# datastax/jvector

Hardware: AMD Instinct MI355X
Metric: QPS@recall10>=0.95 (10Mx768); distances/sec as % HBM roofline (higher is better)
Workload: dtype f32

## Files before the change

jvector_amd/csrc/gs_body.h:

```cpp
#pragma once

#include <cstdint>

#include "gs_params.h"

#ifndef GS_UBR_VAR_LPS
#define GS_UBR_VAR_LPS 1
#endif

namespace jv {

struct alignas(16) gs_f4 { float x, y, z, w; };
struct alignas(16) gs_u4 { uint32_t x, y, z, w; };

GS_FN int32_t gs_float_bits(float f)
{
    int32_t b;
    __builtin_memcpy(&b, &f, 4);
    return b;
}
GS_FN float gs_bits_float(int32_t b)
{
    float f;
    __builtin_memcpy(&f, &b, 4);
// ... 60 lines not shown
    *idx_out = (int)gs_shfl((long long)bi, gs_first(who));
    return m;
}

GS_FN long long gs_scan_top2(const long long *a, int n, int *idx_out, long long *second_out)
{
    const int lane = gs_lane();
    long long best = GS_KEY_MIN, second = GS_KEY_MIN;
    int bi = -1;
    for (int i = lane; i < n; i += 256) {
        long long k[4];
#pragma unroll
        for (int u = 0; u < 4; ++u) k[u] = (i + 64 * u < n) ? a[i + 64 * u] : GS_KEY_MIN;
#pragma unroll
        for (int u = 0; u < 4; ++u) {
            if (k[u] > best) {
                second = best;
                best = k[u];
                bi = i + 64 * u;
            } else if (k[u] > second) {
                second = k[u];
            }
        }
    }
    const long long m = gs_wave_max(best);
    const int w = gs_first(gs_ballot(bi >= 0 && best == m));
    *idx_out = (int)gs_shfl((long long)bi, w);
    *second_out = gs_wave_max(lane == w ? second : best);
    return m;
}

template <int CH16>
GS_FN void gs_load_row(const uint8_t *rp, gs_u4 (&w)[CH16])
{
    const gs_u4 *r4 = reinterpret_cast<const gs_u4 *>(rp);
#pragma unroll
    for (int c = 0; c < CH16; ++c) w[c] = r4[c];
}

template <int VSF, int CH16>
GS_FN float gs_row_sum(const float *codebooks, const float *qs, const gs_u4 (&w)[CH16])
{
    float sum = 0.0f;
#pragma unroll
    for (int c = 0; c < CH16; ++c) {
        const uint32_t d[4] = {w[c].x, w[c].y, w[c].z, w[c].w};
#pragma unroll
        for (int e = 0; e < 4; ++e) {
#pragma unroll
            for (int b = 0; b < 4; ++b) {
                const int m = c * 16 + e * 4 + b;
                const uint32_t code = (d[e] >> (8 * b)) & 0xFFu;
                const gs_f4 *cp = reinterpret_cast<const gs_f4 *>(codebooks + ((int64_t)(m * 256) + code) * 8);
                const gs_f4 c0 = cp[0], c1 = cp[1];
                const float *q = qs + m * 8;
                float ent = 0.0f;
                if (VSF == 0 ) {
                    float t;
                    t = c0.x - q[0]; ent += t * t;
                    t = c0.y - q[1]; ent += t * t;
                    t = c0.z - q[2]; ent += t * t;
                    t = c0.w - q[3]; ent += t * t;
                    t = c1.x - q[4]; ent += t * t;
                    t = c1.y - q[5]; ent += t * t;
                    t = c1.z - q[6]; ent += t * t;
                    t = c1.w - q[7]; ent += t * t;
                } else {
                    ent += c0.x * q[0];
                    ent += c0.y * q[1];
                    ent += c0.z * q[2];
                    ent += c0.w * q[3];
                    ent += c1.x * q[4];
                    ent += c1.y * q[5];
                    ent += c1.z * q[6];
                    ent += c1.w * q[7];
                }
                sum += ent;
            }
        }
    }
    return sum;
}

template <int VSF>
GS_FN float gs_row_sum_any(const GsParams &p, const float *qs, const uint8_t *rp)
{
    float sum = 0.0f;
    const int M = p.M;
    if (p.sub_uniform4 > 0) {
        const int S = p.sub_uniform4;
#pragma unroll 4
        for (int m = 0; m < M; ++m) {
            const gs_f4 *cp = reinterpret_cast<const gs_f4 *>(p.codebooks + ((int64_t)m * 256 + rp[m]) * S);
            const float *q = qs + m * S;
            float ent = 0.0f;
            for (int j = 0; j < S; j += 4) {
                const gs_f4 c = cp[j >> 2];
                if (VSF == 0 ) {
                    float t;
                    t = c.x - q[j]; ent += t * t;
                    t = c.y - q[j + 1]; ent += t * t;
                    t = c.z - q[j + 2]; ent += t * t;
                    t = c.w - q[j + 3]; ent += t * t;
                } else {
                    ent += c.x * q[j];
                    ent += c.y * q[j + 1];
                    ent += c.z * q[j + 2];
                    ent += c.w * q[j + 3];
                }
            }
            sum += ent;
        }
        return sum;
    }
#pragma unroll 2
    for (int m = 0; m < M; ++m) {
        const int S = p.sub_sizes[m];
        const float *cb = p.codebooks + p.cb_offsets[m] + (int64_t)rp[m] * S;
        const float *q = qs + p.sub_offsets[m];
        float ent = 0.0f;
        for (int j = 0; j < S; ++j) {
            if (VSF == 0 ) {
                const float t = cb[j] - q[j];
                ent += t * t;
            } else {
                ent += cb[j] * q[j];
            }
        }
        sum += ent;
    }
    return sum;
}

template <int VSF>
GS_FN float gs_lut_entry_from(const gs_f4 c0, const gs_f4 c1, const float *q);
template <int VSF>
GS_FN float gs_lut_entry(const float *codebooks, const float *qs, int m, int code)
{
    const gs_f4 *cp = reinterpret_cast<const gs_f4 *>(codebooks + ((int64_t)(m * 256) + code) * 8);
    return gs_lut_entry_from<VSF>(cp[0], cp[1], qs + m * 8);
}
template <int VSF>
GS_FN float gs_lut_entry_from(const gs_f4 c0, const gs_f4 c1, const float *q)
{
    float ent = 0.0f;
    if (VSF == 0 ) {
        float t;
        t = c0.x - q[0]; ent += t * t;
        t = c0.y - q[1]; ent += t * t;
        t = c0.z - q[2]; ent += t * t;
        t = c0.w - q[3]; ent += t * t;
        t = c1.x - q[4]; ent += t * t;
        t = c1.y - q[5]; ent += t * t;
        t = c1.z - q[6]; ent += t * t;
        t = c1.w - q[7]; ent += t * t;
    } else {
        ent += c0.x * q[0];
        ent += c0.y * q[1];
        ent += c0.z * q[2];
        ent += c0.w * q[3];
        ent += c1.x * q[4];
        ent += c1.y * q[5];
        ent += c1.z * q[6];
        ent += c1.w * q[7];
    }
    return ent;
}

template <int VSF>
GS_FN float gs_lut_entry_pk(const gs_f4 c0, const gs_f4 c1, const float *q)
{
#ifdef GS_HAVE_PK_F32
    if (VSF != 0) {
        const gs_f4 q0 = reinterpret_cast<const gs_f4 *>(q)[0], q1 = reinterpret_cast<const gs_f4 *>(q)[1];
        const gs_pk2 p01 = gs_pk2{c0.x, c0.y} * gs_pk2{q0.x, q0.y}, p23 = gs_pk2{c0.z, c0.w} * gs_pk2{q0.z, q0.w};
        const gs_pk2 p45 = gs_pk2{c1.x, c1.y} * gs_pk2{q1.x, q1.y}, p67 = gs_pk2{c1.z, c1.w} * gs_pk2{q1.z, q1.w};
        float ent = 0.0f;
        ent += p01.x;
        ent += p01.y;
        ent += p23.x;
        ent += p23.y;
        ent += p45.x;
        ent += p45.y;
        ent += p67.x;
        ent += p67.y;
        return ent;
    }
#endif
    return gs_lut_entry_from<VSF>(c0, c1, q);
}

template <int VSF>
GS_FN float gs_lut_entry_pk_q(const gs_f4 c0, const gs_f4 c1, const gs_f4 q0, const gs_f4 q1)
{
#ifdef GS_HAVE_PK_F32
    if (VSF != 0) {
        const gs_pk2 p01 = gs_pk2{c0.x, c0.y} * gs_pk2{q0.x, q0.y}, p23 = gs_pk2{c0.z, c0.w} * gs_pk2{q0.z, q0.w};
        const gs_pk2 p45 = gs_pk2{c1.x, c1.y} * gs_pk2{q1.x, q1.y}, p67 = gs_pk2{c1.z, c1.w} * gs_pk2{q1.z, q1.w};
        float ent = 0.0f;
        ent += p01.x;
        ent += p01.y;
        ent += p23.x;
        ent += p23.y;
        ent += p45.x;
        ent += p45.y;
        ent += p67.x;
        ent += p67.y;
        return ent;
    }
#endif
    const float q[8] = {q0.x, q0.y, q0.z, q0.w, q1.x, q1.y, q1.z, q1.w};
    return gs_lut_entry_from<VSF>(c0, c1, q);
}

template <int VSF, int CH16, bool FULL = false>
GS_FN float gx_row_sum(const float *lut, int lut_m, const float *codebooks, const float *qs, const gs_u4 (&w)[CH16])
{
    float sum = 0.0f;
#pragma unroll
    for (int c = 0; c < CH16; ++c) {
        const uint32_t d[4] = {w[c].x, w[c].y, w[c].z, w[c].w};
        if (FULL || c * 16 < lut_m) {
#pragma unroll
            for (int e = 0; e < 4; ++e) {
#pragma unroll
                for (int b = 0; b < 4; ++b) {
                    const int m = c * 16 + e * 4 + b;
                    const uint32_t code = (d[e] >> (8 * b)) & 0xFFu;
                    sum += lut[m * 256 + (int)code];
                }
            }
        } else {
#pragma unroll
            for (int e = 0; e < 4; ++e) {
#pragma unroll
                for (int b = 0; b < 4; ++b) {
                    const int m = c * 16 + e * 4 + b;
                    const uint32_t code = (d[e] >> (8 * b)) & 0xFFu;
                    sum += gs_lut_entry<VSF>(codebooks, qs, m, (int)code);
                }
            }
        }
    }
    return sum;
}

struct alignas(8) gs_u2 { uint32_t x, y; };

template <int HW>
GS_FN void gs_load_half(const uint8_t *rp, gs_u2 (&w)[HW])
{
    const gs_u2 *r2 = reinterpret_cast<const gs_u2 *>(rp);
#pragma unroll
    for (int c = 0; c < HW; ++c) w[c] = r2[c];
}

template <int VSF, int HW, int XS = 32>
GS_FN float gs_half_entries(const float *codebooks, const float *qs, const gs_u2 (&w)[HW], int m_base, float *xw)
{
    float sum = 0.0f;
#pragma unroll
    for (int c = 0; c < HW; ++c) {
        const uint32_t d[2] = {w[c].x, w[c].y};
#pragma unroll
        for (int e = 0; e < 2; ++e) {
#pragma unroll
            for (int b = 0; b < 4; ++b) {
                const int j = c * 8 + e * 4 + b;
                const int m = m_base + j;
                const uint32_t code = (d[e] >> (8 * b)) & 0xFFu;
                const gs_f4 *cp = reinterpret_cast<const gs_f4 *>(codebooks + ((int64_t)m * 256 + code) * 8);
                const gs_f4 c0 = cp[0], c1 = cp[1];
                const float *q = qs + m * 8;
                float v = 0.0f;
                if (VSF == 0 ) {
                    float t;
                    t = c0.x - q[0]; v += t * t;
                    t = c0.y - q[1]; v += t * t;
                    t = c0.z - q[2]; v += t * t;
                    t = c0.w - q[3]; v += t * t;
                    t = c1.x - q[4]; v += t * t;
                    t = c1.y - q[5]; v += t * t;
                    t = c1.z - q[6]; v += t * t;
                    t = c1.w - q[7]; v += t * t;
                } else {
                    v += c0.x * q[0];
                    v += c0.y * q[1];
                    v += c0.z * q[2];
                    v += c0.w * q[3];
                    v += c1.x * q[4];
                    v += c1.y * q[5];
                    v += c1.z * q[6];
                    v += c1.w * q[7];
                }
                if (xw) xw[j * XS] = v;
                else sum += v;
            }
        }
    }
    return sum;
}


template <int CH16>
GS_FN void gs_ubr_load(const uint32_t *tab_q, uint32_t (&tab)[CH16 * 16])
{
    const gs_u4 *src = reinterpret_cast<const gs_u4 *>(tab_q) + gs_lane();
#pragma unroll
    for (int k = 0; k < CH16 * 4; ++k) {
        const gs_u4 v = src[k * 64];
        tab[4 * k + 0] = v.x;
        tab[4 * k + 1] = v.y;
        tab[4 * k + 2] = v.z;
        tab[4 * k + 3] = v.w;
    }
}

template <int CH16>
GS_FN int32_t gs_ubr_half(const uint32_t (&tab)[CH16 * 16], const gs_u2 (&w)[CH16], int hi, bool lower = false)
{
    int32_t acc = lower ? 0 : CH16 * 8;
    const uint32_t selbase = 0x0c0c0c00u + 2u * (uint32_t)hi;
#pragma unroll
    for (int c = 0; c < CH16; ++c) {
        const uint32_t d[2] = {w[c].x, w[c].y};
        uint32_t lo[8], up[8], sel[8];
#pragma unroll
        for (int i = 0; i < 8; ++i) {
            const int r = c * 8 + i;
            const uint32_t code = (d[i >> 2] >> (8 * (i & 3))) & 0xFFu;
            const int src = (int)(code & 63u);
            lo[i] = (uint32_t)gs_shfl32((int32_t)tab[2 * r], src);
            up[i] = (uint32_t)gs_shfl32((int32_t)tab[2 * r + 1], src);
            const uint32_t t2 = code >> 6;
            sel[i] = selbase + t2 + (t2 & 2u);
        }
#pragma unroll
        for (int i = 0; i < 8; ++i) acc += (int32_t)gs_perm(up[i], lo[i], sel[i]);
    }
    return acc;
}

template <int VSF>
GS_FN float gs_finish(float sum, float node_mag, float query_mag)
{
    if (VSF == 0) return 1.0f / (1.0f + sum);
    if (VSF == 2) {
        const float prod = node_mag * query_mag;
        sum = (float)((double)sum / gs_sqrt((double)prod));
    }
    return (1.0f + sum) / 2.0f;
}

template <int VSF>
GS_FN bool gs_bound_below(float bound_raw, float node_mag, float query_mag, float T)
{
    if (VSF == 0) return bound_raw > 0.0f && gs_finish<VSF>(bound_raw, node_mag, query_mag) < T;
    if (VSF != 2) return gs_finish<VSF>(bound_raw, node_mag, query_mag) < T;
    const float prod = node_mag * query_mag;
    if (!(prod > 0.0f) || !(prod < 3.0e38f)) return false;
    const float x = bound_raw * gs_rsq_approx(prod);
    const float ax = x < 0.0f ? -x : x;
    return x + 1e-5f * (1.0f + ax) < 2.0f * T - 1.0f;
}

template <int VSF>
GS_FN float gs_bound_score(float bound_raw, float node_mag, float query_mag)
{
    float u;
    if (VSF == 2) {
        const float prod = node_mag * query_mag;
        if (!(prod > 0.0f) || !(prod < 3.0e38f)) return __builtin_inff();
        const float x = bound_raw * gs_rsq_approx(prod);
        const float ax = x < 0.0f ? -x : x;
        u = 0.5f * (1.0f + (x + 1e-5f * (1.0f + ax)));
    } else {
        u = gs_finish<VSF>(bound_raw, node_mag, query_mag);
    }
    const float au = u < 0.0f ? -u : u;
    return u + 1e-6f * (1.0f + au);
}

template <int VSF, int M_, int LPS>
GS_FN void gs_ubr_pass(const float *codebooks, const float *qs, float *xf, const int32_t *st_nb, const float *st_mag, const uint8_t *st_code,
                       int base, int ns, float query_mag, bool ub_active, float ub_T, bool &fresh, long long &key)
{
    static_assert(M_ % LPS == 0 && (LPS == 8 || LPS == 16 || LPS == 32), "lanes per survivor");
    constexpr int SUBS = M_ / LPS;
    constexpr int RH = SUBS % 6 == 0 ? 6 : (SUBS % 4 == 0 ? 4 : SUBS);
    constexpr int QB = RH % 3 == 0 ? 3 : (RH % 2 == 0 ? 2 : 1);
    static_assert(SUBS % RH == 0 && RH % QB == 0 && RH <= 6, "whole rounds of whole batches");
    constexpr int NB = (LPS - 1) * SUBS;
    constexpr int CS = (NB + 3) & ~3;
    const int lane = gs_lane();
    const int g = lane / LPS;
    int t = lane % LPS;
    GS_OPAQUE_I32(t);
    const int j = base + g;
    const bool work = j < ns;
    float sum = 0.0f;
    if (work) {
        const int off = t * SUBS;
        const uint32_t *cw = reinterpret_cast<const uint32_t *>(st_code + j * M_ + (off & ~3));
        uint32_t d[SUBS / 4 > 3 ? SUBS / 4 : 3];
        if (SUBS % 4 == 0) {
#pragma unroll
            for (int i = 0; i < SUBS / 4; ++i) d[i] = cw[i];
        } else {
            const unsigned long long win = (unsigned long long)cw[0] | ((unsigned long long)cw[1] << 32);
            const unsigned long long sh = win >> (8 * (off & 3));
            d[0] = (uint32_t)sh;
            d[1] = (uint32_t)(sh >> 32);
            d[2] = 0u;
        }
        float v[SUBS];
#pragma unroll
        for (int h2 = 0; h2 < SUBS / RH; ++h2) {
            gs_f4 c0[RH], c1[RH];
#pragma unroll
            for (int kk = 0; kk < RH; ++kk) {
                const int k = h2 * RH + kk;
                const uint32_t code = (d[k >> 2] >> (8 * (k & 3))) & 0xFFu;
                const gs_f4 *cp = reinterpret_cast<const gs_f4 *>(codebooks + ((int64_t)((t * SUBS + k) * 256) + code) * 8);
                c0[kk] = cp[0];
                c1[kk] = cp[1];
            }
#pragma unroll
            for (int b3 = 0; b3 < RH / QB; ++b3) {
                gs_f4 q0[QB], q1[QB];
#pragma unroll
                for (int kk = 0; kk < QB; ++kk) {
                    const gs_f4 *qp = reinterpret_cast<const gs_f4 *>(qs + (t * SUBS + h2 * RH + b3 * QB + kk) * 8);
                    q0[kk] = qp[0];
                    q1[kk] = qp[1];
                }
                GS_SCHED_FENCE();
#pragma unroll
                for (int kk = 0; kk < QB; ++kk) {
                    const int k = h2 * RH + b3 * QB + kk;
                    v[k] = gs_lut_entry_pk_q<VSF>(c0[b3 * QB + kk], c1[b3 * QB + kk], q0[kk], q1[kk]);
                }
                GS_SCHED_FENCE();
            }
        }
        if (t == 0) {
#pragma unroll
            for (int k = 0; k < SUBS; ++k) sum += v[k];
        } else {
#pragma unroll
            for (int k = 0; k < SUBS; ++k) xf[g * CS + (t - 1) * SUBS + k] = v[k];
        }
    }
    gs_barrier();
    fresh = work && t == 0;
    key = 0;
    if (fresh) {
        const gs_f4 *col = reinterpret_cast<const gs_f4 *>(xf + g * CS);
        constexpr int NW = CS / 4;
        constexpr int EB = NW % 7 == 0 ? 7 : 8;
#pragma unroll
        for (int b7 = 0; b7 < (NW + EB - 1) / EB; ++b7) {
            gs_f4 e4[EB];
#pragma unroll
            for (int i = 0; i < EB; ++i)
                if (b7 * EB + i < NW) e4[i] = col[b7 * EB + i];
            GS_SCHED_FENCE();
#pragma unroll
            for (int i = 0; i < EB; ++i) {
                const int w0 = (b7 * EB + i) * 4;
                if (w0 + 0 < NB) sum += e4[i].x;
                if (w0 + 1 < NB) sum += e4[i].y;
                if (w0 + 2 < NB) sum += e4[i].z;
                if (w0 + 3 < NB) sum += e4[i].w;
            }
            GS_SCHED_FENCE();
        }
        const float sc = gs_finish<VSF>(sum, st_mag[j], query_mag);
        key = gs_key(st_nb[j], sc);
        if (ub_active && sc < ub_T) fresh = false;
    }
}

GS_FN bool gs_visit(int32_t *tab, uint32_t mask, int shift, int32_t node)
{
    uint32_t h = ((uint32_t)node * 0x9E3779B1u) >> shift;
    for (;;) {
        const int32_t old = gs_cas(tab + h, -1, node);
        if (old == -1) return true;
        if (old == node) return false;
        h = (h + 1) & mask;
    }
}

struct GsVis1 {
    uint32_t *w;
    uint32_t bmask;
    uint32_t idmask;
    int rbits;
};

GS_FN int gs_v1_bucket(uint32_t *bw, uint32_t mine)
{
    for (;;) {
        const uint32_t w0 = bw[0], w1 = bw[1];
        const uint32_t e0 = w0 & 0xFFFFu, e1 = w0 >> 16, e2 = w1 & 0xFFFFu, e3 = w1 >> 16;
        if (e0 == mine || e1 == mine || e2 == mine || e3 == mine) return 0;
        const int slot = e0 == 0xFFFFu ? 0 : (e1 == 0xFFFFu ? 1 : (e2 == 0xFFFFu ? 2 : (e3 == 0xFFFFu ? 3 : -1)));
        if (slot < 0) return 2;
        const uint32_t w = slot < 2 ? w0 : w1;
        const int sh = (slot & 1) * 16;
        const uint32_t want = (w & ~(0xFFFFu << sh)) | (mine << sh);
        if (gs_lds_cas(bw + (slot >> 1), w, want) == w) return 1;
    }
}

GS_FN int gs_visit1(const GsVis1 &t, int32_t node)
{
    const uint32_t rmask = (1u << t.rbits) - 1u;
    const uint32_t h0 = ((uint32_t)node * 0x9E3779B1u) & t.idmask;
    const int r = gs_v1_bucket(t.w + 2u * ((h0 >> t.rbits) & t.bmask), h0 & rmask);
    if (r != 2) return r;
    const uint32_t h1 = ((uint32_t)node * 0x85EBCA6Bu) & t.idmask;
    return gs_v1_bucket(t.w + 2u * ((h1 >> t.rbits) & t.bmask), (1u << t.rbits) | (h1 & rmask));
}

GS_FN const int32_t *gs_level_row(const GsLevel &L, int32_t node)
{
    if (!L.hkeys) return (node >= 0 && node < L.count) ? L.nbrs + (int64_t)node * L.degree : nullptr;
    uint32_t h = ((uint32_t)node * 0x9E3779B1u) >> L.hshift;
    for (;;) {
        const int32_t k = L.hkeys[h];
        if (k == node) return L.nbrs + (int64_t)L.hvals[h] * L.degree;
        if (k == -1) return nullptr;
        h = (h + 1) & L.hmask;
    }
}

struct GsState {
    long long *cand, *res, *evicted, *samp;
    long long *spill;
    int cand_n, spill_n, res_n, ev_n, res_min_idx, spill_cap;
    long long spill_max, res_min;
    int32_t status;
};

GS_FN void gs_partition(GsState &s, const GsParams &p)
{
    const int lane = gs_lane();
    const uint64_t lt = (1ull << lane) - 1ull;
    const long long mine = s.cand[(int)(((long long)lane * s.cand_n) >> 6)];
    s.samp[lane] = mine;
    gs_barrier();
    int rank = 0;
    for (int j = 0; j < 64; ++j) rank += (s.samp[j] < mine) ? 1 : 0;
    const long long pivot = gs_shfl(mine, gs_first(gs_ballot(rank == 31)));
    int new_n = 0, moved = 0;
    for (int base = 0; base < s.cand_n; base += 64) {
        const int i = base + lane;
        const bool in = i < s.cand_n;
        const long long k = in ? s.cand[i] : 0;
        const bool hi = in && k > pivot;
        const bool lo = in && !hi;
        const uint64_t mh = gs_ballot(hi), ml = gs_ballot(lo);
        if (hi) s.cand[new_n + gs_popc(mh & lt)] = k;
        if (lo) {
            const int pos = s.spill_n + moved + gs_popc(ml & lt);
            if (pos < s.spill_cap) s.spill[pos] = k;
        }
        new_n += gs_popc(mh);
        moved += gs_popc(ml);
        gs_barrier();
    }
    if (s.spill_n + moved > s.spill_cap) s.status = GS_OVERFLOW;
    s.spill_n += moved;
    s.cand_n = new_n;
    s.spill_max = pivot;
}

GS_FN void gs_refill(GsState &s, const GsParams &p)
{
    const int lane = gs_lane();
    const uint64_t lt = (1ull << lane) - 1ull;
    gs_fence();
    const int n = s.spill_n;
    if (n <= p.cand_cap / 2) {
        for (int base = 0; base < n; base += 64)
            if (base + lane < n) s.cand[base + lane] = s.spill[base + lane];
        s.cand_n = n;
        s.spill_n = 0;
        s.spill_max = GS_KEY_MIN;
        gs_barrier();
        return;
    }
    const long long mine = s.spill[(int)(((long long)lane * n) >> 6)];
    s.samp[lane] = mine;
    gs_barrier();
    int rank = 0;
    for (int j = 0; j < 64; ++j) rank += (s.samp[j] < mine) ? 1 : 0;
    int r = 63 - (int)(((long long)(p.cand_cap / 4) * 64) / n);
    r = r < 1 ? 1 : (r > 62 ? 62 : r);
    long long pivot = 0;
    int above = 0;
    for (int attempt = 0; attempt < 8; ++attempt) {
        pivot = gs_shfl(mine, gs_first(gs_ballot(rank == r)));
        above = 0;
        for (int base = 0; base < n; base += 64) above += gs_popc(gs_ballot(base + lane < n && s.spill[base + lane] > pivot));
        if (above <= p.cand_cap - 64 || r >= 62) break;
        r += (64 - r) / 2;
        if (r > 62) r = 62;
    }
    gs_barrier();
    if (above == 0 || above > p.cand_cap - 64) return;
    int nc = 0, ns = 0;
    for (int base = 0; base < n; base += 64) {
        const int i = base + lane;
        const bool in = i < n;
        const long long k = in ? s.spill[i] : 0;
        const bool hi = in && k > pivot;
        const bool lo = in && !hi;
        const uint64_t mh = gs_ballot(hi), ml = gs_ballot(lo);
        if (hi) s.cand[nc + gs_popc(mh & lt)] = k;
        if (lo) s.spill[ns + gs_popc(ml & lt)] = k;
        nc += gs_popc(mh);
        ns += gs_popc(ml);
        gs_barrier();
    }
    s.cand_n = nc;
    s.spill_n = ns;
    s.spill_max = pivot;
    gs_fence();
}

GS_FN void gs_push(GsState &s, const GsParams &p, long long key, bool has)
{
    const int lane = gs_lane();
    const uint64_t lt = (1ull << lane) - 1ull;
    bool to_lds;
    uint64_t ml;
    for (;;) {
        to_lds = has && (s.spill_n == 0 || key > s.spill_max);
        ml = gs_ballot(to_lds);
// ... 1236 lines not shown
```

jvector_amd/csrc/gs_wave_hip.h:

```cpp
#pragma once

#include <hip/hip_runtime.h>

#include <cstdint>

#define GS_FN __device__ __forceinline__
#define GS_SCHED_FENCE() __builtin_amdgcn_sched_barrier(0)
#define GS_NOINLINE __device__ __attribute__((noinline))
#define GS_LDS_AS __attribute__((address_space(3)))
#define GS_GLOBAL_AS __attribute__((address_space(1)))
__device__ __forceinline__ int gs_lane() { return (int)threadIdx.x; }
#ifdef GS_WAVE_SCOPE_BARRIER
__device__ __forceinline__ void gs_barrier()
{
    __builtin_amdgcn_fence(__ATOMIC_RELEASE, "wavefront");
    __builtin_amdgcn_wave_barrier();
    __builtin_amdgcn_fence(__ATOMIC_ACQUIRE, "wavefront");
}
#else
__device__ __forceinline__ void gs_barrier() { __syncthreads(); }
#endif
__device__ __forceinline__ int gs_tid() { return (int)threadIdx.x; }
__device__ __forceinline__ void gs_block_barrier() { __syncthreads(); }
__device__ __forceinline__ int gs_block_threads() { return (int)blockDim.x; }
__device__ __forceinline__ int32_t gs_lds_load(const int32_t *p)
{
    const int32_t v = *(const volatile __attribute__((address_space(3))) int32_t *)p;
    __asm__ volatile("s_waitcnt lgkmcnt(0)" ::: "memory");
    return v;
}
__device__ __forceinline__ void gs_lds_store(int32_t *p, int32_t v)
{
    __asm__ volatile("s_waitcnt lgkmcnt(0)" ::: "memory");
    *(volatile __attribute__((address_space(3))) int32_t *)p = v;
}
__device__ __forceinline__ int32_t gs_lds_add(int32_t *p, int32_t v)
{
    return __hip_atomic_fetch_add((__attribute__((address_space(3))) int32_t *)p, v, __ATOMIC_RELAXED, __HIP_MEMORY_SCOPE_WORKGROUP);
}
__device__ __forceinline__ void gs_spin_pause() { __builtin_amdgcn_s_sleep(1); }
__device__ __forceinline__ void gs_sched_fence() { __builtin_amdgcn_sched_barrier(0); }
__device__ __forceinline__ uint64_t gs_ballot(bool p) { return (uint64_t)__ballot(p ? 1 : 0); }
#ifdef GS_UNIFORM_SHFL
__device__ __forceinline__ long long gs_shfl(long long v, int src)
{
    const int lo = __builtin_amdgcn_readlane((int)(unsigned long long)v, src), hi = __builtin_amdgcn_readlane((int)((unsigned long long)v >> 32), src);
    return (long long)(((unsigned long long)(unsigned)hi << 32) | (unsigned long long)(unsigned)lo);
}
#define GS_HAVE_WAVE_REDUCE 1
template <bool MAX>
__device__ __forceinline__ long long gs_wave_reduce64(long long v)
{
#define JV_DPP_STEP(CTRL, ROWS)                                                                                       \
    do {                                                                                                              \
        const int lo_ = __builtin_amdgcn_update_dpp((int)(unsigned long long)v, (int)(unsigned long long)v, CTRL, ROWS, 0xf, false);              \
        const int hi_ = __builtin_amdgcn_update_dpp((int)((unsigned long long)v >> 32), (int)((unsigned long long)v >> 32), CTRL, ROWS, 0xf, false); \
        const long long o_ = (long long)(((unsigned long long)(unsigned)hi_ << 32) | (unsigned long long)(unsigned)lo_);                          \
        v = MAX ? (o_ > v ? o_ : v) : (o_ < v ? o_ : v);                                                              \
    } while (0)
    JV_DPP_STEP(0x111, 0xf);
    JV_DPP_STEP(0x112, 0xf);
    JV_DPP_STEP(0x114, 0xf);
    JV_DPP_STEP(0x118, 0xf);
    JV_DPP_STEP(0x142, 0xa);
    JV_DPP_STEP(0x143, 0xc);
#undef JV_DPP_STEP
    const int lo = __builtin_amdgcn_readlane((int)(unsigned long long)v, 63), hi = __builtin_amdgcn_readlane((int)((unsigned long long)v >> 32), 63);
    return (long long)(((unsigned long long)(unsigned)hi << 32) | (unsigned long long)(unsigned)lo);
}
__device__ __forceinline__ long long gs_wave_max(long long v) { return gs_wave_reduce64<true>(v); }
__device__ __forceinline__ long long gs_wave_min(long long v) { return gs_wave_reduce64<false>(v); }
#define GS_HAVE_WAVE_REDUCE32 1
#define JV_DPP_RED32(T, NAME, EXPR)                                                                  \
    __device__ __forceinline__ T NAME(T v)                                                           \
    {                                                                                                \
        _Pragma("unroll") for (int s_ = 0; s_ < 6; ++s_)                                             \
        {                                                                                            \
            T o_;                                                                                    \
            switch (s_) {                                                                            \
            case 0: o_ = (T)__builtin_amdgcn_update_dpp((int)v, (int)v, 0x111, 0xf, 0xf, false); break; \
            case 1: o_ = (T)__builtin_amdgcn_update_dpp((int)v, (int)v, 0x112, 0xf, 0xf, false); break; \
            case 2: o_ = (T)__builtin_amdgcn_update_dpp((int)v, (int)v, 0x114, 0xf, 0xf, false); break; \
            case 3: o_ = (T)__builtin_amdgcn_update_dpp((int)v, (int)v, 0x118, 0xf, 0xf, false); break; \
            case 4: o_ = (T)__builtin_amdgcn_update_dpp((int)v, (int)v, 0x142, 0xa, 0xf, false); break; \
            default: o_ = (T)__builtin_amdgcn_update_dpp((int)v, (int)v, 0x143, 0xc, 0xf, false); break; \
            }                                                                                        \
            v = EXPR;                                                                                \
        }                                                                                            \
        return (T)__builtin_amdgcn_readlane((int)v, 63);                                             \
    }
JV_DPP_RED32(int32_t, gs_wave_max_i32, (o_ > v ? o_ : v))
JV_DPP_RED32(int32_t, gs_wave_min_i32, (o_ < v ? o_ : v))
JV_DPP_RED32(uint32_t, gs_wave_max_u32, (o_ > v ? o_ : v))
#undef JV_DPP_RED32
__device__ __forceinline__ int32_t gs_uniform(int32_t v) { return __builtin_amdgcn_readfirstlane(v); }
#else
__device__ __forceinline__ long long gs_shfl(long long v, int src) { return __shfl(v, src, 64); }
#endif
__device__ __forceinline__ uint32_t gs_bcast32(uint32_t v, int src) { return (uint32_t)__builtin_amdgcn_readlane((int)v, src); }
__device__ __forceinline__ long long gs_shfl_xor(long long v, int m) { return __shfl_xor(v, m, 64); }
#define GS_OPAQUE_I32(x) asm volatile("" : "+v"(x))
__device__ __forceinline__ int32_t gs_shfl32(int32_t v, int src) { return __builtin_amdgcn_ds_bpermute(src << 2, v); }
#define GS_HAVE_PK_F32 1
typedef float gs_pk2 __attribute__((ext_vector_type(2)));
__device__ __forceinline__ uint32_t gs_perm(uint32_t hi, uint32_t lo, uint32_t sel) { return __builtin_amdgcn_perm(hi, lo, sel); }
__device__ __forceinline__ int32_t gs_cas(int32_t *p, int32_t expect, int32_t desired) { return atomicCAS(p, expect, desired); }
__device__ __forceinline__ uint32_t gs_lds_cas(uint32_t *p, uint32_t expect, uint32_t desired)
{
    typedef __attribute__((address_space(3))) uint32_t lds_u32;
    lds_u32 *lp = (lds_u32 *)p;
    __hip_atomic_compare_exchange_strong(lp, &expect, desired, __ATOMIC_RELAXED, __ATOMIC_RELAXED, __HIP_MEMORY_SCOPE_WORKGROUP);
    return expect;
}
__device__ __forceinline__ void gs_prefetch_lds(const void *g, void *lds)
{
    typedef __attribute__((address_space(1))) const void gptr;
    typedef __attribute__((address_space(3))) void lptr;
    __builtin_amdgcn_global_load_lds((gptr *)g, (lptr *)lds, 4, 0, 0);
}
__device__ __forceinline__ uint32_t gs_fetch_add(uint32_t *p, uint32_t v) { return atomicAdd(p, v); }
__device__ __forceinline__ void gs_fetch_add64(unsigned long long *p, unsigned long long v) { (void)atomicAdd(p, v); }
#define GS_CLOCK() ((unsigned long long)__builtin_readcyclecounter())
__device__ __forceinline__ void gs_fence() { __threadfence(); }
__device__ __forceinline__ double gs_sqrt(double x) { return sqrt(x); }
__device__ __forceinline__ float gs_rsq_approx(float x) { return __builtin_amdgcn_rsqf(x); }
typedef float gs_f32x16 __attribute__((ext_vector_type(16)));
__device__ __forceinline__ gs_f32x16 gs_mfma_32x32x2(float a, float b, gs_f32x16 c)
{
    return __builtin_amdgcn_mfma_f32_32x32x2f32(a, b, c, 0, 0, 0);
}
__device__ __forceinline__ float gs_fmaf(float a, float b, float c) { return __builtin_fmaf(a, b, c); }
__device__ __forceinline__ void gs_gather64(float v, float (&out)[64])
{
#pragma unroll
    for (int i = 0; i < 64; ++i) out[i] = __builtin_bit_cast(float, __builtin_amdgcn_readlane(__builtin_bit_cast(int, v), i));
}
```

Before: 2.552 million.

## Regroup UBR table halves at load and feed raw codes to bpermute addresses

The quantized lookup table is rearranged once at load time with byte-perm instructions so that each 16-bit entry pair is grouped differently. This lets the inner lookup loop pass shifted code bytes directly as ds_bpermute byte addresses, since bpermute ignores the high address bits, and build the perm selector with a single mask and OR instead of per-code extract, add and mask work. The 64-bit wave min/max reduction is also rewritten as a 32-bit reduction on the high word plus a ballot-based tie resolution on the low word. The changes cut ALU work in the hot distance loop, and an opaque barrier on the accumulator constrains scheduling. The risk is correctness of the new selector and layout mapping, plus the extra conditional path in the reduction.

```diff
diff --git a/jvector_amd/csrc/gs_body.h b/jvector_amd/csrc/gs_body.h
--- a/jvector_amd/csrc/gs_body.h
+++ b/jvector_amd/csrc/gs_body.h
@@ -386,13 +386,28 @@
 }
 
 
+#ifndef GS_HAVE_SHFL32_ADDR
+GS_FN int32_t gs_shfl32_addr(int32_t v, uint32_t addr) { return gs_shfl32(v, (int)((addr >> 2) & 63u)); }
+#endif
+
+#ifndef GS_HAVE_REGROUP16
+GS_FN void gs_regroup16(uint32_t &a, uint32_t &b)
+{
+    const uint32_t x = gs_perm(b, a, 0x05040100u), y = gs_perm(b, a, 0x07060302u);
+    a = x;
+    b = y;
+}
+#endif
+
 template <int CH16>
 GS_FN void gs_ubr_load(const uint32_t *tab_q, uint32_t (&tab)[CH16 * 16])
 {
     const gs_u4 *src = reinterpret_cast<const gs_u4 *>(tab_q) + gs_lane();
 #pragma unroll
     for (int k = 0; k < CH16 * 4; ++k) {
-        const gs_u4 v = src[k * 64];
+        gs_u4 v = src[k * 64];
+        gs_regroup16(v.x, v.y);
+        gs_regroup16(v.z, v.w);
         tab[4 * k + 0] = v.x;
         tab[4 * k + 1] = v.y;
         tab[4 * k + 2] = v.z;
@@ -404,23 +419,23 @@
 GS_FN int32_t gs_ubr_half(const uint32_t (&tab)[CH16 * 16], const gs_u2 (&w)[CH16], int hi, bool lower = false)
 {
     int32_t acc = lower ? 0 : CH16 * 8;
-    const uint32_t selbase = 0x0c0c0c00u + 2u * (uint32_t)hi;
+    const uint32_t selbase = 0x0c0c0c00u + 4u * (uint32_t)hi;
 #pragma unroll
     for (int c = 0; c < CH16; ++c) {
         const uint32_t d[2] = {w[c].x, w[c].y};
-        uint32_t lo[8], up[8], sel[8];
+        const uint32_t q6[2] = {(d[0] >> 6) & 0x03030303u, (d[1] >> 6) & 0x03030303u};
+        uint32_t x[8], y[8], sel[8];
 #pragma unroll
         for (int i = 0; i < 8; ++i) {
-            const int r = c * 8 + i;
-            const uint32_t code = (d[i >> 2] >> (8 * (i & 3))) & 0xFFu;
-            const int src = (int)(code & 63u);
-            lo[i] = (uint32_t)gs_shfl32((int32_t)tab[2 * r], src);
-            up[i] = (uint32_t)gs_shfl32((int32_t)tab[2 * r + 1], src);
-            const uint32_t t2 = code >> 6;
-            sel[i] = selbase + t2 + (t2 & 2u);
-        }
-#pragma unroll
-        for (int i = 0; i < 8; ++i) acc += (int32_t)gs_perm(up[i], lo[i], sel[i]);
+            const int r = c * 8 + i, b = i & 3;
+            const uint32_t addr = b == 0 ? d[i >> 2] << 2 : d[i >> 2] >> (8 * b - 2);
+            x[i] = (uint32_t)gs_shfl32_addr((int32_t)tab[2 * r], addr);
+            y[i] = (uint32_t)gs_shfl32_addr((int32_t)tab[2 * r + 1], addr);
+            sel[i] = selbase | ((q6[i >> 2] >> (8 * b)) & 0xFFu);
+        }
+#pragma unroll
+        for (int i = 0; i < 8; ++i) acc += (int32_t)gs_perm(y[i], x[i], sel[i]);
+        GS_OPAQUE_I32(acc);
     }
     return acc;
 }
diff --git a/jvector_amd/csrc/gs_wave_hip.h b/jvector_amd/csrc/gs_wave_hip.h
--- a/jvector_amd/csrc/gs_wave_hip.h
+++ b/jvector_amd/csrc/gs_wave_hip.h
@@ -47,29 +47,6 @@
     const int lo = __builtin_amdgcn_readlane((int)(unsigned long long)v, src), hi = __builtin_amdgcn_readlane((int)((unsigned long long)v >> 32), src);
     return (long long)(((unsigned long long)(unsigned)hi << 32) | (unsigned long long)(unsigned)lo);
 }
-#define GS_HAVE_WAVE_REDUCE 1
-template <bool MAX>
-__device__ __forceinline__ long long gs_wave_reduce64(long long v)
-{
-#define JV_DPP_STEP(CTRL, ROWS)                                                                                       \
-    do {                                                                                                              \
-        const int lo_ = __builtin_amdgcn_update_dpp((int)(unsigned long long)v, (int)(unsigned long long)v, CTRL, ROWS, 0xf, false);              \
-        const int hi_ = __builtin_amdgcn_update_dpp((int)((unsigned long long)v >> 32), (int)((unsigned long long)v >> 32), CTRL, ROWS, 0xf, false); \
-        const long long o_ = (long long)(((unsigned long long)(unsigned)hi_ << 32) | (unsigned long long)(unsigned)lo_);                          \
-        v = MAX ? (o_ > v ? o_ : v) : (o_ < v ? o_ : v);                                                              \
-    } while (0)
-    JV_DPP_STEP(0x111, 0xf);
-    JV_DPP_STEP(0x112, 0xf);
-    JV_DPP_STEP(0x114, 0xf);
-    JV_DPP_STEP(0x118, 0xf);
-    JV_DPP_STEP(0x142, 0xa);
-    JV_DPP_STEP(0x143, 0xc);
-#undef JV_DPP_STEP
-    const int lo = __builtin_amdgcn_readlane((int)(unsigned long long)v, 63), hi = __builtin_amdgcn_readlane((int)((unsigned long long)v >> 32), 63);
-    return (long long)(((unsigned long long)(unsigned)hi << 32) | (unsigned long long)(unsigned)lo);
-}
-__device__ __forceinline__ long long gs_wave_max(long long v) { return gs_wave_reduce64<true>(v); }
-__device__ __forceinline__ long long gs_wave_min(long long v) { return gs_wave_reduce64<false>(v); }
 #define GS_HAVE_WAVE_REDUCE32 1
 #define JV_DPP_RED32(T, NAME, EXPR)                                                                  \
     __device__ __forceinline__ T NAME(T v)                                                           \
@@ -92,7 +69,24 @@
 JV_DPP_RED32(int32_t, gs_wave_max_i32, (o_ > v ? o_ : v))
 JV_DPP_RED32(int32_t, gs_wave_min_i32, (o_ < v ? o_ : v))
 JV_DPP_RED32(uint32_t, gs_wave_max_u32, (o_ > v ? o_ : v))
+JV_DPP_RED32(uint32_t, gs_wave_min_u32, (o_ < v ? o_ : v))
 #undef JV_DPP_RED32
+#define GS_HAVE_WAVE_REDUCE 1
+template <bool MAX>
+__device__ __forceinline__ long long gs_wave_reduce64(long long v)
+{
+    const int32_t hi = (int32_t)((unsigned long long)v >> 32);
+    const uint32_t lo = (uint32_t)(unsigned long long)v;
+    const int32_t rh = MAX ? gs_wave_max_i32(hi) : gs_wave_min_i32(hi);
+    const bool tie = hi == rh;
+    const unsigned long long tm = __ballot(tie ? 1 : 0);
+    uint32_t rl;
+    if (tm & (tm - 1ull)) rl = MAX ? gs_wave_max_u32(tie ? lo : 0u) : gs_wave_min_u32(tie ? lo : 0xFFFFFFFFu);
+    else rl = (uint32_t)__builtin_amdgcn_readlane((int)lo, __builtin_ctzll(tm));
+    return (long long)(((unsigned long long)(uint32_t)rh << 32) | (unsigned long long)rl);
+}
+__device__ __forceinline__ long long gs_wave_max(long long v) { return gs_wave_reduce64<true>(v); }
+__device__ __forceinline__ long long gs_wave_min(long long v) { return gs_wave_reduce64<false>(v); }
 __device__ __forceinline__ int32_t gs_uniform(int32_t v) { return __builtin_amdgcn_readfirstlane(v); }
 #else
 __device__ __forceinline__ long long gs_shfl(long long v, int src) { return __shfl(v, src, 64); }
@@ -101,6 +95,16 @@
 __device__ __forceinline__ long long gs_shfl_xor(long long v, int m) { return __shfl_xor(v, m, 64); }
 #define GS_OPAQUE_I32(x) asm volatile("" : "+v"(x))
 __device__ __forceinline__ int32_t gs_shfl32(int32_t v, int src) { return __builtin_amdgcn_ds_bpermute(src << 2, v); }
+#define GS_HAVE_SHFL32_ADDR 1
+__device__ __forceinline__ int32_t gs_shfl32_addr(int32_t v, uint32_t addr) { return __builtin_amdgcn_ds_bpermute((int)addr, v); }
+#define GS_HAVE_REGROUP16 1
+__device__ __forceinline__ void gs_regroup16(uint32_t &a, uint32_t &b)
+{
+    uint32_t t;
+    asm volatile("v_perm_b32 %2, %1, %0, %3\n\tv_perm_b32 %0, %1, %0, %4\n\tv_mov_b32 %1, %2"
+                 : "+v"(a), "+v"(b), "=&v"(t)
+                 : "s"(0x07060302u), "s"(0x05040100u));
+}
 #define GS_HAVE_PK_F32 1
 typedef float gs_pk2 __attribute__((ext_vector_type(2)));
 __device__ __forceinline__ uint32_t gs_perm(uint32_t hi, uint32_t lo, uint32_t sel) { return __builtin_amdgcn_perm(hi, lo, sel); }
```

New measurement: 2.570 million (median of 6 runs). About the same (+0.7%).
